# jorr3/Alphazero-4-player-chess

Measured on AMD Instinct MI355X. Metric: MCTS simulations/sec (whole node), 256 games×400 sims, 10-block ResNet, higher is better.
Workload: dtype fp16

## Files before the change

alphazero-4-player-chess_amd/csrc/fpc_fc.h:

```cpp
#pragma once
#include <hip/hip_runtime.h>

#include <type_traits>

#include "fpc_tower.h"

namespace fpc {

struct FcArgs {
  const uint16_t *X;
  const uint16_t *Wf;
  float *part;
  int Kp, Np, ksteps, Mtot;
  int G1, s1, s2;
  const int *n_live;
};

constexpr int FC_THREADS = 256;
constexpr int FC_XBUF = 256 * 64 * 2;
constexpr int FC_WRING = 16 * 1024;
constexpr int FC_LDS = 3 * FC_XBUF + 4 * FC_WRING;

__device__ __forceinline__ void fc_dma(const void *gsrc_uniform, uint32_t lane_off, uint32_t lds_addr_uniform) {
  uint32_t keep;
// ... 173 lines not shown
  f32x4_t acc[16][6];
  u32x4_t xr[4], wf[2][6];
  const std::integral_constant<int, 0> c0{};
  const std::integral_constant<int, 1> c1{};

  auto issue_x = [&](int s, int p) {
    const int sc = s < S ? s : S - 1;
    fc_dma(xbase + (long)p * xpiece + (long)sc * 128, xlane[p & 1],
           (uint32_t)__builtin_amdgcn_readfirstlane((s & 1) * FC_XBUF + (wave * 64 + p * 8) * 128));
  };
  auto issue_w2 = [&](int s, int j, int n0) {
    const int sc = s < S ? s : S - 1;
    fc_dma2_nt(wbase + (long)(2 * sc + j) * wk32 + n0 * 1024, wlane,
               (uint32_t)__builtin_amdgcn_readfirstlane(lds_w + ((s & 1) * 12 + j * 6 + n0) * 1024));
  };
  auto xfrag = [&](int slot, int t, const unsigned char *ab, int j) {
    xr[slot] = *reinterpret_cast<const u32x4_t *>(ab + lds_off<64>(t * 16 + (lane & 15), j * 4 + (lane >> 4)));
  };
  auto wfrag = [&](int b, int s, int j) {
#pragma unroll
    for (int n = 0; n < 6; ++n) wf[b][n] = *reinterpret_cast<const u32x4_t *>(wr + ((s & 1) * 12 + j * 6 + n) * 1024);
  };
  auto kstep = [&](auto j_c, auto z_c, int s) {
    constexpr int J = decltype(j_c)::value;
    constexpr bool Z = decltype(z_c)::value != 0;
    constexpr int CUR = J, NXT = J ^ 1;
    asm volatile("s_waitcnt vmcnt(20)" ::: "memory");
    const unsigned char *ab = smem + (s & 1) * FC_XBUF;
    const unsigned char *abn = J == 1 ? smem + ((s + 1) & 1) * FC_XBUF : ab;
    __builtin_amdgcn_sched_barrier(0);
    wfrag(NXT, J == 1 ? s + 1 : s, NXT);
    __builtin_amdgcn_sched_barrier(0);
#pragma unroll
    for (int t = 0; t < 16; ++t) {
#pragma unroll
      for (int n = 0; n < 6; ++n) {
        if (n < 4) fcw_mfma<DT, true, Z>(acc[t][n], wf[CUR][n], xr[t & 3]);
        else fcw_mfma<DT, false, Z>(acc[t][n], wf[CUR][n], xr[t & 3]);
      }
      __builtin_amdgcn_sched_barrier(0);
      if (J == 1 && t == 13) { asm volatile("s_waitcnt vmcnt(12)" ::: "memory"); __syncthreads(); }
      if (t + 3 < 16) xfrag((t + 3) & 3, t + 3, ab, J);
      else xfrag((t + 3) & 3, t + 3 - 16, abn, NXT);
      if (J == 0 && t < 8) issue_x(s + 1, t);
      if (J == 0 && (t == 8 || t == 10 || t == 12)) issue_w2(s + 2, 0, t - 8);
      if (J == 1 && (t == 2 || t == 6 || t == 10)) issue_w2(s + 2, 1, (t - 2) / 2);
      __builtin_amdgcn_sched_barrier(0);
    }
  };

#pragma unroll
  for (int p = 0; p < 8; ++p) issue_x(0, p);
#pragma unroll
  for (int st = 0; st < 2; ++st)
#pragma unroll
    for (int j = 0; j < 2; ++j) { issue_w2(st, j, 0); issue_w2(st, j, 2); issue_w2(st, j, 4); }
  asm volatile("s_waitcnt vmcnt(0)" ::: "memory");
  __syncthreads();
#pragma unroll
  for (int t = 0; t < 3; ++t) xfrag(t, t, smem, 0);
  wfrag(0, 0, 0);

  kstep(c0, c1, 0);
  kstep(c1, c0, 0);
#pragma unroll 1
  for (int s = 1; s < S; ++s) {
    kstep(c0, c0, s);
    kstep(c1, c0, s);
  }
  asm volatile("s_waitcnt vmcnt(0)" ::: "memory");
  asm volatile("s_nop 7\n\ts_nop 7\n\ts_nop 3" ::: "memory");

  float *out = g.part + ((long)id * g.Mtot + mrow0) * FCW_COLS;
#pragma unroll
  for (int t = 0; t < 16; ++t) {
    const int m = t * 16 + (lane & 15);
#pragma unroll
    for (int n = 0; n < 6; ++n)
      *reinterpret_cast<f32x4_t *>(out + (long)m * FCW_COLS + wave * 96 + n * 16 + (lane >> 4) * 4) = acc[t][n];
  }
}


template <bool LIVE = false>
__global__ void __launch_bounds__(256) k_fc_reduce(const float *part, const float *bias, int G1, int s1, int s2, int gw, int Mtot, int A,
                                                   int n_rows, const int *n_live, float *logits, float *stats) {
  __shared__ float red[8];
  const int q = blockIdx.x * 256 + threadIdx.x;
  const int m = blockIdx.y;
  if (m >= n_rows || (LIVE && m >= *n_live)) return;
  const bool valid = q * 4 < A;
  float4 v{0.f, 0.f, 0.f, 0.f};
  if (valid) {
    const int j = gw == 256 ? q >> 6 : (q * 4) / gw;
    const int col = q * 4 - j * gw;
    const int base = j < G1 ? j * s1 : G1 * s1 + (j - G1) * s2, cnt = j < G1 ? s1 : s2;
    v = *reinterpret_cast<const float4 *>(bias + q * 4);
    for (int k = 0; k < cnt; ++k) {
      const float4 p = *reinterpret_cast<const float4 *>(part + ((long)(base + k) * Mtot + m) * gw + col);
      v.x += p.x; v.y += p.y; v.z += p.z; v.w += p.w;
    }
    if (logits) *reinterpret_cast<float4 *>(logits + (long)m * A + q * 4) = v;
  }
  softmax_chunk_stats(v, valid, red, stats + ((long)m * SM_MAXCH + blockIdx.x) * SM_REC);
}

}
```

alphazero-4-player-chess_amd/csrc/fpc_nn.h:

```cpp
#pragma once
#include <hip/hip_runtime.h>

#include <algorithm>
#include <cstdlib>
#include <cstring>
#include <string>
#include <vector>

#include "fpc_tree_kernels.h"
#include "fpc_pack.h"
#include "fpc_tower.h"
#include "fpc_towerw.h"

namespace fpc {

typedef __attribute__((ext_vector_type(8))) __bf16 bf16x8_t;
typedef __attribute__((ext_vector_type(8))) _Float16 f16x8_t;
typedef __attribute__((ext_vector_type(16))) float f32x16_t;
typedef __attribute__((ext_vector_type(4))) uint32_t u32x4_t;
typedef __attribute__((ext_vector_type(2))) uint32_t u32x2_t;
typedef __attribute__((ext_vector_type(4))) float f32x4_t;

template <int DT>
struct E16;
// ... 276 lines not shown
            const u32x4_t x = xrow[q0 + 64 * u];
            a0 = Dot16<DT>::dot2(w[u][0], x[0], a0); a1 = Dot16<DT>::dot2(w[u][1], x[1], a1);
            a2 = Dot16<DT>::dot2(w[u][2], x[2], a2); a3 = Dot16<DT>::dot2(w[u][3], x[3], a3);
          }
        }
      }
      float a = (a0 + a1) + (a2 + a3);
      for (int off = 32; off >= 1; off >>= 1) a += __shfl_xor(a, off);
      if (lane == 0) ll[(size_t)g * FPC_MAX_MOVES + j] = bias[nsrc] + a;
    }
    p = pend;
  }
}

template <int DT>
__global__ void __launch_bounds__(64) k_value_tail(const uint16_t *Y, const float *w, float bias, int P, int R, int PP,
                                                   int n, float *out) {
  const int g = blockIdx.x;
  if (g >= n) return;
  const int lane = threadIdx.x & 63;
  float acc = 0.f;
  for (int idx = lane; idx < R * R * 32; idx += 64) {
    const int q = idx >> 5, ch = idx & 31;
    const long m = (long)g * PP + (q / R + 1) * P + (q % R + 1);
    acc += E16<DT>::to_f32(Y[m * 32 + ch]) * w[idx];
  }
  for (int off = 32; off >= 1; off >>= 1) acc += __shfl_xor(acc, off);
  if (lane == 0) out[g] = tanhf(acc + bias);
}

template <int DT>
__global__ void __launch_bounds__(64) k_nchw_to_grid(const float *x, int n, int R, int P, uint16_t *out) {
  const int g = blockIdx.x;
  if (g >= n) return;
  const int lane = threadIdx.x & 63, RR = R * R;
  for (int q = lane; q < RR; q += 64) {
    uint16_t *row = out + ((long)g * P * P + (q / R + 1) * P + (q % R + 1)) * 32;
    for (int c = 0; c < 32; ++c) row[c] = c < 24 ? E16<DT>::from_f32(x[((long)g * 24 + c) * RR + q]) : (uint16_t)0;
  }
}

struct BlobHeader {
  char magic[4];
  int32_t version, R, F, nblocks, dtype, A_ch, Np, Kp;
  int32_t fc_layout;
  int32_t pad[6];
};
static_assert(sizeof(BlobHeader) == 64, "header is 64 bytes");

struct ConvW {
  uint16_t *w = nullptr;
  float *b = nullptr;
  int cin = 0, cout_pad = 0;
};

struct NN {
  bool loaded = false;
  DevCfg dc{};
  int Gmax = 0, dtype = 0, F = 0, nblocks = 0, P = 0, PP = 0, Np = 0, Kp = 0, Mrows = 0, guard = 64, Gpad = 0;
  hipStream_t stream = nullptr;
  std::vector<void *> allocs;
  uint16_t *in16 = nullptr;
  uint16_t *act[3] = {nullptr, nullptr, nullptr};
  uint16_t *yv = nullptr;
  uint16_t *xfc = nullptr;
  float *d_logits = nullptr;
  float *d_stats = nullptr;
  float *d_value = nullptr;
  ConvW stem, pconv, vconv;
  std::vector<ConvW> c1, c2;
  uint16_t *fcw = nullptr;
  float *fcb = nullptr, *vw = nullptr;
  float *fc_part = nullptr;
  int fc_G1 = 0, fc_s1 = FC_SPLITK, fc_s2 = FC_SPLITK;
  int fc_layout = 1;
  int fc_gw = 256;
  unsigned char *towerW = nullptr;
  unsigned char *stemW = nullptr;
  float *towerB = nullptr;
  bool use_tower = false;
  int tower_waves = 8;
  bool tower_compact = true;
  bool tower_taploop = true;
  int towerw_rows = 1;
  bool use_towerw = false;
  void (*mark_fn)(void *, int) = nullptr;
  void *mark_ctx = nullptr;
  float vb = 0.f;
  bool attr_conv[2][3] = {{false, false, false}, {false, false, false}}, attr_tower[2] = {false, false}, attr_towerw[2] = {false, false}, attr_fc[2] = {false, false}, attr_gemv = false;

  template <class T>
  int dmalloc(T **p, size_t count, std::string *err) {
    void *q = nullptr;
    if (hipMalloc(&q, count * sizeof(T)) != hipSuccess) { *err = "hipMalloc failed in NN (" + std::to_string(count * sizeof(T)) + " bytes)"; return FPC_ENOMEM; }
    (void)hipMemset(q, 0, count * sizeof(T));
    allocs.push_back(q);
    *p = (T *)q;
    return 0;
  }

  int init(const DevCfg &c, int max_games, int nn_dtype, hipStream_t s, std::string *) {
    dc = c; Gmax = max_games; dtype = nn_dtype ? 1 : 0; stream = s;
    P = c.R + 2; PP = P * P;
    Mrows = ((max_games * PP + CONV_BM - 1) / CONV_BM) * CONV_BM;
    Gpad = ((max_games + 255) / 256) * 256;
    return 0;
  }
  void destroy() {
    for (void *p : allocs) (void)hipFree(p);
    allocs.clear();
    loaded = false;
    fcw2 = nullptr; d_ll = nullptr;
  }
  uint16_t *input16() { return in16 + (size_t)guard * 32; }
  const fpc_board *in_boards = nullptr;
  const int *in_leaf_slot = nullptr, *in_leaf_turn = nullptr;
  int in_board_stride = 0;
  bool takes_boards() const { return use_tower || use_towerw; }
  void set_board_input(const fpc_board *b, int stride, const int *slot, const int *turn) { in_boards = b; in_board_stride = stride; in_leaf_slot = slot; in_leaf_turn = turn; }
  const int *in_live_count = nullptr;
  void set_live_count(const int *n_live) { in_live_count = n_live; }
  uint16_t one16() const { return dtype ? 0x3C00 : 0x3F80; }
  float *logits() { return d_logits; }
  float *stats() { return d_stats; }
  float *value() { return d_value; }
  uint16_t *fcw2 = nullptr;
  float *d_ll = nullptr;
  float *legal_logits() { return d_ll; }

  static int plan_fcw(int Np, int Kp, int cus) { return pk_plan_fcw(Np, Kp, cus); }
  static_assert(PK_FCW_COLS == FCW_COLS && PK_FCW_MAXSPLIT == 2 * FC_SPLITK, "fpc_pack.h plans k_fcw's split with these");
  void plan_fc() {
    if (fc_layout == 2) { fc_G1 = Np / FCW_COLS; fc_s2 = fc_s1; return; }
    fc_s1 = FC_SPLITK;
    const int groups = Np / 256, ks = Kp / 16, mt = (Gmax + 255) / 256;
    fc_s2 = (ks % (2 * FC_SPLITK * 8) == 0 && ks / (2 * FC_SPLITK) / 4 >= 4) ? 2 * FC_SPLITK : FC_SPLITK;
    fc_G1 = groups;
    if (fc_s2 == FC_SPLITK) return;
    int cus = 256;
    hipDeviceProp_t prop;
    int dev = 0;
    (void)hipGetDevice(&dev);
    if (hipGetDeviceProperties(&prop, dev) == hipSuccess && prop.multiProcessorCount > 0) cus = prop.multiProcessorCount;
    long best = -1;
    std::vector<long> fin(cus);
    for (int g1 = groups; g1 >= 0; --g1) {
      std::fill(fin.begin(), fin.end(), 0L);
      for (int y = 0; y < mt; ++y)
        for (int id = 0, nb = g1 * FC_SPLITK + (groups - g1) * fc_s2; id < nb; ++id) {
          auto it = std::min_element(fin.begin(), fin.end());
          *it += id < g1 * FC_SPLITK ? 2 : 1;
        }
      const long span = *std::max_element(fin.begin(), fin.end());
      if (best < 0 || span < best) { best = span; fc_G1 = g1; }
    }
  }

  static int device_cus() {
    int cus = 256, dev = 0;
    hipDeviceProp_t prop;
    (void)hipGetDevice(&dev);
    if (hipGetDeviceProperties(&prop, dev) == hipSuccess && prop.multiProcessorCount > 0) cus = prop.multiProcessorCount;
    return cus;
  }
  int check_geom(int gF, int gnblocks, int gNp, int gKp, int glayout, int *split, std::string *err) const {
    return pk_check_geom(gF, gnblocks, gNp, gKp, glayout, dc.A, device_cus(), split, err);
  }
  bool same_geom(int gF, int gnblocks, int gNp, int gKp, int glayout) const {
    return loaded && F == gF && nblocks == gnblocks && Np == gNp && Kp == gKp && fc_layout == glayout;
  }
  int alloc_net(int gF, int gnblocks, int gNp, int gKp, int glayout, int split, std::string *err) {
    destroy();
    F = gF; nblocks = gnblocks; Np = gNp; Kp = gKp;
    fc_layout = glayout;
    fc_gw = fc_layout == 2 ? FCW_COLS : 256;
    if (fc_layout == 2) fc_s1 = split;
    int rc = 0;
    auto conv = [&](ConvW &cw, int cin, int cout_pad) -> int {
      cw.cin = cin; cw.cout_pad = cout_pad;
      if ((rc = dmalloc(&cw.w, (size_t)9 * cout_pad * cin, err))) return rc;
      return dmalloc(&cw.b, (size_t)cout_pad, err);
    };
    const int Fp = (F + GEMM_BN - 1) / GEMM_BN * GEMM_BN;
    if ((rc = conv(stem, 32, Fp))) return rc;
    c1.assign(nblocks, ConvW()); c2.assign(nblocks, ConvW());
    for (int i = 0; i < nblocks; ++i) { if ((rc = conv(c1[i], F, Fp)) || (rc = conv(c2[i], F, Fp))) return rc; }
    if ((rc = conv(pconv, F, 128))) return rc;
    if ((rc = conv(vconv, F, 128))) return rc;
    if ((rc = dmalloc(&fcw, (size_t)Np * Kp, err)) || (rc = dmalloc(&fcb, (size_t)Np, err))) return rc;
    if ((rc = dmalloc(&vw, (size_t)dc.RR * 32, err))) return rc;
    const size_t rows = (size_t)Mrows + 2 * guard;
    if ((rc = dmalloc(&in16, rows * 32, err))) return rc;
    for (auto &a : act) if ((rc = dmalloc(&a, rows * F, err))) return rc;
    if ((rc = dmalloc(&yv, rows * 32, err))) return rc;
    if ((rc = dmalloc(&xfc, (size_t)Gpad * Kp, err))) return rc;
    if ((rc = dmalloc(&fc_part, (size_t)2 * FC_SPLITK * Gpad * Np, err))) return rc;
    plan_fc();
    if ((rc = dmalloc(&d_logits, (size_t)Gmax * dc.A, err))) return rc;
    if ((rc = dmalloc(&d_stats, (size_t)Gmax * SM_MAXCH * SM_REC, err))) return rc;
    if ((rc = dmalloc(&d_value, (size_t)Gmax, err))) return rc;
    use_tower = use_towerw = false;
    const bool dev = getenv("FPC_DEV_KNOBS") && atoi(getenv("FPC_DEV_KNOBS")) != 0;
    auto knob = [dev](const char *name, int dflt) { const char *v = dev ? getenv(name) : nullptr; return v ? atoi(v) : dflt; };
    const bool no_tower = knob("FPC_NO_TOWER", 0) != 0;
    tower_waves = knob("FPC_TOWER_WAVES", 8);
    tower_compact = knob("FPC_TOWER_COMPACT", 1) != 0;
    tower_taploop = knob("FPC_TOWER_TAPLOOP", 1) != 0;
    if (F == 256 && !no_tower) {
      use_towerw = true;
      towerw_rows = knob("FPC_TOWERW_ROWS", 1);
    } else if (F == 128 && !no_tower) {
      const int kw = knob("FPC_TOWERW", -1);
      use_towerw = kw < 0 ? dc.R != 14 : kw != 0;
      use_tower = !use_towerw;
    }
    const int layers = 2 * nblocks + 2;
    if (use_towerw) {
      const int slab = tww_slab(F), ksn = F / 32;
      if ((rc = dmalloc(&towerW, ((size_t)layers * 9 * ksn + TWW_PAD_SLABS) * slab, err)) || (rc = dmalloc(&stemW, (size_t)9 * slab, err)) ||
          (rc = dmalloc(&towerB, (size_t)layers * 256, err))) return rc;
    } else if (use_tower) {
      if ((rc = dmalloc(&towerW, (size_t)(layers * 9 + 3) * TW_TAP, err)) || (rc = dmalloc(&stemW, (size_t)9 * TW_STEM_TAP, err)) ||
          (rc = dmalloc(&towerB, (size_t)layers * 256, err))) return rc;
    }
    return 0;
  }
  std::vector<ConvW *> convs_in_blob_order() {
    std::vector<ConvW *> v{&stem};
    for (int i = 0; i < nblocks; ++i) { v.push_back(&c1[i]); v.push_back(&c2[i]); }
    v.push_back(&pconv); v.push_back(&vconv);
    return v;
  }
  int finish_weights(std::string *err) {
    if (use_towerw) {
      const int slab = tww_slab(F), ksn = F / 32, tiles = F / 16;
      auto prep = [&](const ConvW &cw, int layer) {
        hipLaunchKernelGGL(k_towerw_prep, dim3((9 * ksn * tiles * 64 + 255) / 256), dim3(256), 0, stream, (const uint16_t *)cw.w,
                           towerW + (size_t)layer * 9 * ksn * slab, 9, cw.cout_pad, F, tiles);
        (void)hipMemcpyAsync(towerB + (size_t)layer * 256, cw.b, (size_t)std::min(cw.cout_pad, F) * 4, hipMemcpyDeviceToDevice, stream);
      };
      for (int i = 0; i < nblocks; ++i) { prep(c1[i], 2 * i); prep(c2[i], 2 * i + 1); }
      prep(vconv, 2 * nblocks);
      prep(pconv, 2 * nblocks + 1);
      hipLaunchKernelGGL(k_towerw_prep, dim3((9 * tiles * 64 + 255) / 256), dim3(256), 0, stream, (const uint16_t *)stem.w, stemW, 9, stem.cout_pad, 32, tiles);
    } else if (use_tower) {
      auto prep = [&](const ConvW &cw, int layer) {
        hipLaunchKernelGGL(k_tower_prep, dim3((9 * 128 * 16 + 255) / 256), dim3(256), 0, stream, (const uint16_t *)cw.w,
                           towerW + (size_t)layer * 9 * TW_TAP, 9, 128);
        (void)hipMemcpyAsync(towerB + (size_t)layer * 256, cw.b, 128 * 4, hipMemcpyDeviceToDevice, stream);
      };
      for (int i = 0; i < nblocks; ++i) { prep(c1[i], 2 * i); prep(c2[i], 2 * i + 1); }
      prep(vconv, 2 * nblocks);
      prep(pconv, 2 * nblocks + 1);
      hipLaunchKernelGGL(k_tower_prep, dim3((9 * 128 * 4 + 255) / 256), dim3(256), 0, stream, (const uint16_t *)stem.w, stemW, 9, 32);
    }
    if (fcw2) launch_unfrag();
    if (hipStreamSynchronize(stream) != hipSuccess || hipGetLastError() != hipSuccess) { *err = use_towerw ? "k_towerw_prep failed" : use_tower ? "k_tower_prep failed" : "weight load failed"; return FPC_ENODEVICE; }
    loaded = true;
    return 0;
  }

  int load(const void *blob, uint64_t nbytes, std::string *err) {
    if (nbytes < sizeof(BlobHeader)) { *err = "weight blob too small"; return FPC_EWEIGHTS; }
    BlobHeader h;
    memcpy(&h, blob, sizeof(h));
    if (memcmp(h.magic, "FPCW", 4) || h.version != 3) { *err = "bad weight blob magic/version (this engine reads version 3; version 2 carried the retired 32x32x16 policy-Linear order: export again)"; return FPC_EWEIGHTS; }
    if (h.R != dc.R || h.A_ch != dc.A_ch) { *err = "weight blob is for a different board size"; return FPC_EWEIGHTS; }
    if (h.dtype != dtype) { *err = "weight blob dtype differs from engine nn_dtype"; return FPC_EWEIGHTS; }
    int fcw_split = 0, rc = 0;
    if ((rc = check_geom(h.F, h.nblocks, h.Np, h.Kp, h.fc_layout, &fcw_split, err))) return rc;
    if ((rc = alloc_net(h.F, h.nblocks, h.Np, h.Kp, h.fc_layout, fcw_split, err))) return rc;
    const unsigned char *base = (const unsigned char *)blob;
    uint64_t off = sizeof(BlobHeader);
    auto take = [&](void *dev, uint64_t bytes) -> int {
      off = (off + 63) & ~63ull;
      if (off + bytes > nbytes) { *err = "weight blob truncated"; return FPC_EWEIGHTS; }
      if (hipMemcpy(dev, base + off, bytes, hipMemcpyHostToDevice) != hipSuccess) { *err = "weight upload failed"; return FPC_ENODEVICE; }
      off += bytes;
      return 0;
    };
    for (ConvW *cw : convs_in_blob_order())
      if ((rc = take(cw->w, (uint64_t)9 * cw->cout_pad * cw->cin * 2)) || (rc = take(cw->b, (uint64_t)cw->cout_pad * 4))) return rc;
    if ((rc = take(fcw, (uint64_t)Np * Kp * 2)) || (rc = take(fcb, (uint64_t)Np * 4))) return rc;
    if ((rc = take(vw, (uint64_t)dc.RR * 32 * 4))) return rc;
    off = (off + 63) & ~63ull;
    if (off + 4 > nbytes) { *err = "weight blob truncated"; return FPC_EWEIGHTS; }
    memcpy(&vb, base + off, 4);
    return finish_weights(err);
  }

// ... 79 lines not shown
#undef FPC_TWW_ATTR1
          aw = true;
        }
        const int mtw = tww_mt(dc.R);
        if (mtw < 2 || mtw > 7) { *err = "k_towerw: board size outside 8..14"; return FPC_EINVAL; }
#define FPC_TWW_GO(F_, MT_) hipLaunchKernelGGL((k_towerw<DT, F_, MT_>), dim3(n), dim3(TWW_THREADS), tww_lds(F_), stream, t)
#define FPC_TWW_GOS(F_) switch (mtw) { case 2: FPC_TWW_GO(F_, 2); break; case 3: FPC_TWW_GO(F_, 3); break; case 4: FPC_TWW_GO(F_, 4); break; \
                                       case 5: FPC_TWW_GO(F_, 5); break; case 6: FPC_TWW_GO(F_, 6); break; default: FPC_TWW_GO(F_, 7); break; }
        const int tiles = tww_tiles(dc.R);
        const bool onerow = tiles <= 4 || (F == 256 && towerw_rows != 2);
#define FPC_TWW_GO1(F_, MT_) hipLaunchKernelGGL((k_towerw<DT, F_, MT_, true>), dim3(n), dim3(TWW_THREADS), tww_lds(F_), stream, t)
        if (onerow && F == 128) FPC_TWW_GO1(128, 4);
        else if (onerow) {
          switch (tiles) {
            case 4: FPC_TWW_GO1(256, 4); break;   case 6: FPC_TWW_GO1(256, 6); break;   case 7: FPC_TWW_GO1(256, 7); break;
            case 8: FPC_TWW_GO1(256, 8); break;   case 9: FPC_TWW_GO1(256, 9); break;   case 11: FPC_TWW_GO1(256, 11); break;
            default: FPC_TWW_GO1(256, 13); break;
          }
        } else if (F == 256) { FPC_TWW_GOS(256) } else { FPC_TWW_GOS(128) }
#undef FPC_TWW_GO1
#undef FPC_TWW_GOS
#undef FPC_TWW_GO
      } else if (mt == 3 && tower_waves == 8) hipLaunchKernelGGL((k_tower<DT, 3, false, 8>), dim3(n), dim3(512), TW_LDS, stream, t);
      else if (mt == 3) hipLaunchKernelGGL((k_tower<DT, 3, false, 4>), dim3(n), dim3(256), TW_LDS, stream, t);
      else if (mt == 5 && tower_waves == 8) hipLaunchKernelGGL((k_tower<DT, 5, false, 8>), dim3(n), dim3(512), TW_LDS, stream, t);
      else if (mt == 5) hipLaunchKernelGGL((k_tower<DT, 5, false, 4>), dim3(n), dim3(256), TW_LDS, stream, t);
      else if (P != 16 && tower_waves == 8) hipLaunchKernelGGL((k_tower<DT, 7, false, 8>), dim3(n), dim3(512), TW_LDS, stream, t);
      else if (P != 16) hipLaunchKernelGGL((k_tower<DT, 7, false, 4>), dim3(n), dim3(256), TW_LDS, stream, t);
      else if (tower_waves == 8 && tower_compact && dc.R == 14 && tower_taploop) hipLaunchKernelGGL((k_towerc<DT, true>), dim3(n), dim3(512), TW_LDS, stream, t);
      else if (tower_waves == 8 && tower_compact && dc.R == 14) hipLaunchKernelGGL((k_towerc<DT, false>), dim3(n), dim3(512), TW_LDS, stream, t);
      else if (tower_waves == 8) hipLaunchKernelGGL((k_tower<DT, 7, true, 8>), dim3(n), dim3(512), TW_LDS, stream, t);
      else hipLaunchKernelGGL((k_tower<DT, 7, true, 4>), dim3(n), dim3(256), TW_LDS, stream, t);
      const hipError_t le = hipGetLastError();
      if (le != hipSuccess) { *err = std::string("k_tower launch failed: ") + hipGetErrorString(le); return FPC_ENODEVICE; }
#if defined(TW_STAMPS) || defined(TWW_STAMPS)
      if (getenv("FPC_TW_STAMPS_FILE")) {
        unsigned long long h[2 * 8 * 16];
        (void)hipStreamSynchronize(stream);
        (void)hipMemcpy(h, t.stamps, sizeof(h), hipMemcpyDeviceToHost);
        if (FILE *f = fopen(getenv("FPC_TW_STAMPS_FILE"), "w")) {
          for (int i = 0; i < 2 * 8 * 16; ++i) fprintf(f, "%llu%c", h[i], i % 16 == 15 ? '\n' : ' ');
          fclose(f);
        }
      }
#endif
    } else if ((rc = conv(stem, in16, 32, nullptr, act[0], F, F, 0))) return rc;
    const bool fused = use_tower || use_towerw;
    for (int i = 0; i < nblocks && !fused; ++i) {
      const int t1 = (cur + 1) % 3, t2 = (cur + 2) % 3;
      if ((rc = conv(c1[i], act[cur], F, nullptr, act[t1], F, F, 0))) return rc;
      if ((rc = conv(c2[i], act[t1], F, act[cur], act[t2], F, F, 0))) return rc;
      cur = t2;
    }
    if (!fused) {
      if ((rc = conv(pconv, act[cur], F, nullptr, xfc, Kp, dc.A_ch, 1))) return rc;
      if ((rc = conv(vconv, act[cur], F, nullptr, yv, 32, 24, 0))) return rc;
    }
    if (mark_fn) mark_fn(mark_ctx, 2);
#if defined(TW_STRIP) && (TW_STRIP & 128)
    if (false) {
#else
    if (logits_out) {
#endif
      FcArgs f{};
      f.X = xfc; f.Wf = fcw; f.part = fc_part; f.Kp = Kp; f.Np = Np; f.ksteps = Kp / 16; f.Mtot = Gpad;
      f.G1 = fc_G1; f.s1 = fc_s1; f.s2 = fc_s2;
      f.n_live = in_live_count;
      const int mtiles = (n + 255) / 256;
      const int blocks = fc_G1 * fc_s1 + (Np / fc_gw - fc_G1) * fc_s2;
      bool &fattr = attr_fc[DT];
      if (!fattr) {
        (void)hipFuncSetAttribute(reinterpret_cast<const void *>(&k_fc16<DT>), hipFuncAttributeMaxDynamicSharedMemorySize, FC_LDS);
        (void)hipFuncSetAttribute(reinterpret_cast<const void *>(&k_fcw<DT>), hipFuncAttributeMaxDynamicSharedMemorySize, FCW_LDS);
        (void)hipFuncSetAttribute(reinterpret_cast<const void *>(&k_fc16<DT, true>), hipFuncAttributeMaxDynamicSharedMemorySize, FC_LDS);
        (void)hipFuncSetAttribute(reinterpret_cast<const void *>(&k_fcw<DT, true>), hipFuncAttributeMaxDynamicSharedMemorySize, FCW_LDS);
        fattr = true;
      }
      const bool live = in_live_count != nullptr;
      if (fc_layout == 2 && live) hipLaunchKernelGGL((k_fcw<DT, true>), dim3(blocks, mtiles), dim3(FC_THREADS), FCW_LDS, stream, f);
      else if (fc_layout == 2) hipLaunchKernelGGL((k_fcw<DT>), dim3(blocks, mtiles), dim3(FC_THREADS), FCW_LDS, stream, f);
      else if (live) hipLaunchKernelGGL((k_fc16<DT, true>), dim3(blocks, mtiles), dim3(FC_THREADS), FC_LDS, stream, f);
      else hipLaunchKernelGGL((k_fc16<DT>), dim3(blocks, mtiles), dim3(FC_THREADS), FC_LDS, stream, f);
      float *const dense_out = skip_dense ? (float *)nullptr : logits_out;
      if (live)
        hipLaunchKernelGGL(k_fc_reduce<true>, dim3((dc.A / 4 + 255) / 256, n), dim3(256), 0, stream, (const float *)fc_part, (const float *)fcb,
                           fc_G1, fc_s1, fc_s2, fc_gw, Gpad, dc.A, n, in_live_count, dense_out, d_stats);
      else
        hipLaunchKernelGGL(k_fc_reduce<false>, dim3((dc.A / 4 + 255) / 256, n), dim3(256), 0, stream, (const float *)fc_part, (const float *)fcb,
                           fc_G1, fc_s1, fc_s2, fc_gw, Gpad, dc.A, n, in_live_count, dense_out, d_stats);
      const hipError_t le = hipGetLastError();
      if (le != hipSuccess) { *err = std::string("k_fc launch failed: ") + hipGetErrorString(le); return FPC_ENODEVICE; }
    }
    if (!fused) hipLaunchKernelGGL((k_value_tail<DT>), dim3(n), dim3(64), 0, stream, (const uint16_t *)(yv + (size_t)guard * 32),
                       (const float *)vw, vb, P, dc.R, PP, n, value_out);
    if (hipGetLastError() != hipSuccess) { *err = "k_value_tail launch failed"; return FPC_ENODEVICE; }
    return 0;
  }

  bool skip_dense = false;
  int forward(int n, bool dense_logits, std::string *err) {
    skip_dense = !dense_logits;
    const int rc = dtype ? forward_t<1>(n, d_logits, d_value, err) : forward_t<0>(n, d_logits, d_value, err);
    skip_dense = false;
    return rc;
  }
  static_assert(2 * FC_SPLITK <= LOGIT_MAX_SLABS, "logit_at() requests at most LOGIT_MAX_SLABS slabs per column");
  LogitSrc logit_src(bool dense) const {
    if (dense) return LogitSrc{d_logits, nullptr, nullptr, 0, 0, 0, 0, 256};
    return LogitSrc{nullptr, fc_part, fcb, fc_G1, fc_s1, fc_s2, Gpad, fc_gw};
  }
  void launch_unfrag() {
    const long chunks = (long)Np * (Kp / 8);
    if (dtype) hipLaunchKernelGGL((k_fc_unfrag<1>), dim3((unsigned)((chunks + 255) / 256)), dim3(256), 0, stream, (const uint16_t *)fcw, fcw2, Np, Kp);
    else hipLaunchKernelGGL((k_fc_unfrag<0>), dim3((unsigned)((chunks + 255) / 256)), dim3(256), 0, stream, (const uint16_t *)fcw, fcw2, Np, Kp);
  }
  int ensure_legal_head(std::string *err) {
    if (fcw2) return 0;
    if (Gmax > GEMV_MAXG) { *err = "legal-only policy head supports at most " + std::to_string(GEMV_MAXG) + " games per engine"; return FPC_EINVAL; }
    int rc;
    if ((rc = dmalloc(&fcw2, (size_t)Np * Kp, err)) || (rc = dmalloc(&d_ll, (size_t)Gmax * FPC_MAX_MOVES, err))) return rc;
    launch_unfrag();
    if (hipGetLastError() != hipSuccess) { *err = "k_fc_unfrag launch failed"; return FPC_ENODEVICE; }
    return 0;
  }
  int forward_legal(int n, const Tree &t, std::string *err) {
    int rc = ensure_legal_head(err);
    if (rc) return rc;
    if ((rc = dtype ? forward_t<1>(n, nullptr, d_value, err) : forward_t<0>(n, nullptr, d_value, err))) return rc;
    const size_t lds = (size_t)Kp * 2;
    bool &attr = attr_gemv;
    if (!attr) {
      (void)hipFuncSetAttribute(reinterpret_cast<const void *>(&k_policy_gemv<0>), hipFuncAttributeMaxDynamicSharedMemorySize, 64 * 1024);
      (void)hipFuncSetAttribute(reinterpret_cast<const void *>(&k_policy_gemv<1>), hipFuncAttributeMaxDynamicSharedMemorySize, 64 * 1024);
      attr = true;
    }
    if (lds > 64 * 1024) { *err = "legal-only policy head: activation row does not fit LDS"; return FPC_EINVAL; }
    const int blocks = 768;
    if (dtype) hipLaunchKernelGGL((k_policy_gemv<1>), dim3(blocks), dim3(GEMV_THREADS), lds, stream, dc, t, n, (const uint16_t *)xfc, (const uint16_t *)fcw2, (const float *)fcb, Kp, d_ll);
    else hipLaunchKernelGGL((k_policy_gemv<0>), dim3(blocks), dim3(GEMV_THREADS), lds, stream, dc, t, n, (const uint16_t *)xfc, (const uint16_t *)fcw2, (const float *)fcb, Kp, d_ll);
    if (hipGetLastError() != hipSuccess) { *err = "k_policy_gemv launch failed"; return FPC_ENODEVICE; }
    return 0;
  }
  int forward_external(const float *enc, int n, float *logits_out, float *value_out, std::string *err) {
    if (dtype) hipLaunchKernelGGL((k_nchw_to_grid<1>), dim3(n), dim3(64), 0, stream, enc, n, dc.R, P, input16());
    else hipLaunchKernelGGL((k_nchw_to_grid<0>), dim3(n), dim3(64), 0, stream, enc, n, dc.R, P, input16());
    int rc = dtype ? forward_t<1>(n, logits_out, value_out, err) : forward_t<0>(n, logits_out, value_out, err);
    if (rc) return rc;
    if (hipStreamSynchronize(stream) != hipSuccess) { *err = "NN forward failed"; return FPC_ENODEVICE; }
    return 0;
  }
};

}
```

alphazero-4-player-chess_amd/csrc/fpc_tower.h:

```cpp
#pragma once
#include <hip/hip_runtime.h>

#include <type_traits>

#include "fpc_tree_kernels.h"

namespace fpc {

typedef __attribute__((ext_vector_type(8))) __bf16 t_bf16x8;
typedef __attribute__((ext_vector_type(8))) _Float16 t_f16x8;
typedef __attribute__((ext_vector_type(4))) float t_f32x4;
typedef __attribute__((ext_vector_type(2))) float t_f32x2;
typedef __attribute__((ext_vector_type(4))) uint32_t t_u32x4;
typedef __attribute__((ext_vector_type(2))) uint32_t t_u32x2;
typedef __attribute__((ext_vector_type(2))) short t_i16x2;

template <int DT>
struct M16;
template <>
struct M16<0> {
  static __device__ __forceinline__ t_f32x4 mfma(t_u32x4 a, t_u32x4 b, t_f32x4 c) {
    return __builtin_amdgcn_mfma_f32_16x16x32_bf16(__builtin_bit_cast(t_bf16x8, a), __builtin_bit_cast(t_bf16x8, b), c, 0, 0, 0);
  }
  static __device__ __forceinline__ uint32_t pack2(float lo, float hi) {
// ... 74 lines not shown
}
__device__ __forceinline__ void tw_dma_4k(const unsigned char *gsrc_uniform, uint32_t lane_off, uint32_t lds_addr_uniform) {
  uint32_t keep;
  asm volatile(
      "s_mov_b32 %0, m0\n\ts_mov_b32 m0, %3\n\ts_nop 0\n\t"
      "global_load_lds_dwordx4 %1, %2\n\ts_add_u32 m0, m0, 0x400\n\tv_add_u32 %1, 0x400, %1\n\t"
      "global_load_lds_dwordx4 %1, %2\n\ts_add_u32 m0, m0, 0x400\n\tv_add_u32 %1, 0x400, %1\n\t"
      "global_load_lds_dwordx4 %1, %2\n\ts_add_u32 m0, m0, 0x400\n\tv_add_u32 %1, 0x400, %1\n\t"
      "global_load_lds_dwordx4 %1, %2\n\t"
      "s_mov_b32 m0, %0"
      : "=&s"(keep), "+v"(lane_off) : "s"(gsrc_uniform), "s"(lds_addr_uniform) : "memory", "scc");
}
template <int OFF>
__device__ __forceinline__ void tw_dma_piece(const unsigned char *gsrc_uniform, uint32_t lane_off) {
  asm volatile("global_load_lds_dwordx4 %0, %1 offset:%2" : : "v"(lane_off), "s"(gsrc_uniform), "i"(OFF) : "memory");
}
__device__ __forceinline__ void tw_set_m0(uint32_t lds_addr_uniform) {
  asm volatile("s_mov_b32 m0, %0\n\ts_nop 0" : : "s"(lds_addr_uniform) : "memory");
}
__device__ __forceinline__ void tw_dma_256(const unsigned char *gsrc_uniform, uint32_t lane_off, uint32_t lds_addr_uniform) {
  uint32_t keep;
  asm volatile("s_mov_b32 %0, m0\n\ts_mov_b32 m0, %3\n\ts_nop 0\n\tglobal_load_lds_dword %1, %2\n\ts_mov_b32 m0, %0"
               : "=&s"(keep) : "v"(lane_off), "s"(gsrc_uniform), "s"(lds_addr_uniform) : "memory");
}

#ifdef TW_STAMPS
#define TW_STAMP(GT, I)                                                                                       \
  do {                                                                                                        \
    if (g.stamps && blockIdx.x == 0 && ((GT) == TW_STAMPS || (GT) == TW_STAMPS + 1)) {                        \
      const unsigned long long t_ = __builtin_amdgcn_s_memtime();                                             \
      if (lane == 0) g.stamps[(((GT) - TW_STAMPS) * 8 + wave) * 16 + (I)] = t_;                               \
    }                                                                                                         \
  } while (0)
#else
#define TW_STAMP(GT, I) do {} while (0)
#endif
#ifndef TW_AHEAD
#define TW_AHEAD 2
#endif
#ifndef TW_LOADERS
#define TW_LOADERS 1
#endif
#ifndef TW_STAGGER
#define TW_STAGGER 3
#endif
#ifndef TW_STRIP
#define TW_STRIP 0
#endif
#ifndef TWC_LOADER_TILES
#define TWC_LOADER_TILES 6
#endif

#ifndef TWC_STAGGER
#define TWC_STAGGER 2
#endif

template <int DT, int MT, bool FAST, int NW, int LOAD, bool CMP = false, bool TU = false>
__device__ __forceinline__ void tw_body(const TowerArgs &g) {
  static_assert(!CMP || (!FAST && NW == 8 && TW_LOADERS == 1 && MT == (LOAD == 2 ? TWC_LOADER_TILES : 13 - TWC_LOADER_TILES)), "compact form: 8 waves, 13 row tiles");
  static_assert(!TU || (CMP && TW_STAGGER != 0 && TWC_STAGGER >= 1 && TWC_STAGGER <= 3), "tap-specialised loop: compact form with the burst stream");
  constexpr int CR = 14, CZ = 16;
  constexpr int TB0 = LOAD == 2 ? 0 : TWC_LOADER_TILES;
  constexpr int NT = NW * 64;
  constexpr int WN = NW / 2;
  constexpr int CT = 8 / WN;
  constexpr int PIECES = 4 * LOAD;
  constexpr int DMA_PER_WAVE = PIECES * 1024;
  constexpr int MID = PIECES == 8 ? 4096 : 0;
  constexpr bool STREAM = TW_AHEAD == 2 && !(TW_STAGGER != 0 && NW == 8 && TW_LOADERS == 1);
  constexpr int STAG = (NW == 8 && TW_LOADERS == 1 && LOAD == 0) ? (TU ? TWC_STAGGER : TW_STAGGER) : 0;
  extern __shared__ __attribute__((aligned(16))) unsigned char smem[];
  unsigned char *const img = smem + TW_IMG0;
  unsigned char *const ring = smem + TW_RING;
  const float *const biasbuf = reinterpret_cast<const float *>(smem + TW_BIAS);
  float *const vred = reinterpret_cast<float *>(smem + TW_VRED);
  fpc_board *const lboard = reinterpret_cast<fpc_board *>(smem + TW_BOARD);
  const int tid = threadIdx.x, lane = tid & 63;
  const int wave = __builtin_amdgcn_readfirstlane(tid >> 6);
  const int wm = wave / WN, wn = wave % WN;
  const int li = lane & 15, lq = lane >> 4;
  const int game = blockIdx.x;
  const int P = g.P, NR = g.NR;

  int slot = 0, rot_k = 0;
  if (g.boards) {
    slot = g.leaf_slot[game];
    if (slot < 0) return;
    rot_k = first_leaf_turn(g.leaf_slot, g.leaf_turn, g.n_games);
  }

  const int rbase = CMP ? CZ + TB0 * 16 + li : (g.T0 + wm * MT) * 16 + li;
  uint32_t inmask = 0;
#pragma unroll
  for (int mt = 0; mt < MT; ++mt) {
    const int r = rbase + 16 * mt;
    if (CMP) {
      if (r - CZ < CR * CR) inmask |= 1u << mt;
    } else {
      const int pi = r / P, pj = r - pi * P;
      if (r < g.PP && pi >= 1 && pi <= g.R && pj >= 1 && pj <= g.R) inmask |= 1u << mt;
    }
  }
  auto colmask = [](int mt, int dx) -> uint64_t {
    uint32_t m16 = 0;
    for (int i = 0; i < 16; ++i)
      if (dx != 0 && ((TB0 + mt) * 16 + i) % CR == (dx < 0 ? 0 : CR - 1)) m16 |= 1u << i;
    const uint32_t m32 = m16 * 0x10001u;
    return ((uint64_t)m32 << 32) | m32;
  };
  auto lane_select = [](uint32_t a, uint32_t b, uint64_t m) -> uint32_t {
    uint32_t r;
    asm("v_cndmask_b32_e64 %0, %1, %2, %3" : "=v"(r) : "v"(a), "v"(b), "s"(m));
    return r;
  };
  const int bq = (lq >> 1) * 256 + (lq & 1) * 128;
  const int apart = (li >> 3) * 2048 + (li & 7) * 16 + bq;
  const int apart_s = (li >> 3) * 512 + (li & 7) * 16 + bq;
  const int cb64 = wn * (CT * 16);
  const int cb16 = (wn & 1) * 16;
  const bool vactive = wn < 2;

  for (int c = tid; c < (TW_IMG0 + TW_IMG) / 16; c += NT) reinterpret_cast<t_u32x4 *>(smem)[c] = t_u32x4{0u, 0u, 0u, 0u};
  unsigned char *const enc = smem + TW_ENC;
  const int enc_bytes = CMP ? 240 * 64 : ((NR + 7) >> 3) * 512;
  for (int c = tid; c < enc_bytes / 16; c += NT) reinterpret_cast<t_u32x4 *>(enc)[c] = t_u32x4{0u, 0u, 0u, 0u};
  {
    const t_u32x4 *src = reinterpret_cast<const t_u32x4 *>(g.Wstem);
    t_u32x4 *dst = reinterpret_cast<t_u32x4 *>(ring);
    for (int c = tid; c < 9 * TW_STEM_TAP / 16; c += NT) dst[c] = src[c];
  }
  t_f32x4 bst[CT];
#pragma unroll
  for (int ct = 0; ct < CT; ++ct) bst[ct] = *reinterpret_cast<const t_f32x4 *>(g.bstem + cb64 + ct * 16 + 4 * lq);
  __syncthreads();
  if (g.boards) {
    constexpr int WPB = (int)(sizeof(fpc_board) / 4);
    if (tid < WPB) reinterpret_cast<uint32_t *>(lboard)[tid] =
        reinterpret_cast<const uint32_t *>(g.boards + (size_t)game * g.board_stride + slot)[tid];
    __syncthreads();
    if (g.rules & FPC_RULES_ROTATION) rot_k = lboard->turn;
    for (int r = tid; r < (CMP ? CR * CR : g.PP); r += NT) {
      const int pi = CMP ? r / CR + 1 : r / P, pj = CMP ? r % CR + 1 : r - pi * P;
      if (pi < 1 || pi > g.R || pj < 1 || pj > g.R) continue;
      const uint8_t p = lboard->sq[rot90_src(g.R, rot_k, pi - 1, pj - 1)];
      if (!present(p)) continue;
      const int plane = piece_plane(p, lboard->turn, g.rules);
      *reinterpret_cast<uint16_t *>(enc + tw_lay(4, CMP ? CZ + r : r, plane >> 3) + (plane & 7) * 2) = g.one16;
    }
  } else if (CMP) {
    const uint16_t *src = g.in16 + (size_t)game * g.PP * 32;
    for (int c = tid; c < CR * CR * 4; c += NT) {
      const int q = c >> 2, j = c & 3;
      *reinterpret_cast<t_u32x4 *>(enc + tw_lay(4, CZ + q, j)) =
          *reinterpret_cast<const t_u32x4 *>(src + ((size_t)(q / CR + 1) * P + q % CR + 1) * 32 + j * 8);
    }
  } else {
    const uint16_t *src = g.in16 + (size_t)game * g.PP * 32;
    for (int c = tid; c < NR * 4; c += NT) {
      const int r = c >> 2, j = c & 3;
      *reinterpret_cast<t_u32x4 *>(enc + tw_lay(4, r, j)) = *reinterpret_cast<const t_u32x4 *>(src + (size_t)r * 32 + j * 8);
    }
  }
  __syncthreads();

  t_f32x4 acc[MT][CT];
  t_u32x2 res[MT][CT];

  auto brow = [&](int mt, int shift) -> int {
    int r = rbase + 16 * mt + shift;
    r = r < 0 ? r + NR : r;
    r = r >= NR ? r - NR : r;
    return r;
  };

#pragma unroll
  for (int tap = 0; tap < 9; ++tap) {
    const int shift = (tap / 3 - 1) * (CMP ? CR : P) + (tap % 3 - 1);
    t_u32x4 fa[CT], fb[MT];
#pragma unroll
    for (int ct = 0; ct < CT; ++ct)
      fa[ct] = *reinterpret_cast<const t_u32x4 *>(ring + tap * TW_STEM_TAP + (cb64 + ct * 16) * 64 + apart_s);
#pragma unroll
    for (int mt = 0; mt < MT; ++mt) {
      const int r = CMP ? (int)lane_select((uint32_t)(rbase + 16 * mt + shift), (uint32_t)((rbase + shift) & 7), colmask(mt, tap % 3 - 1)) : brow(mt, shift);
      fb[mt] = *reinterpret_cast<const t_u32x4 *>(enc + (r >> 3) * 512 + (r & 7) * 16 + bq);
    }
#pragma unroll
    for (int mt = 0; mt < MT; ++mt)
#pragma unroll
      for (int ct = 0; ct < CT; ++ct) acc[mt][ct] = M16<DT>::mfma(fa[ct], fb[mt], tap == 0 ? bst[ct] : acc[mt][ct]);
  }
  __syncthreads();

  const int total = (g.L + 2) * 9;
  const uint32_t dma_lane = (uint32_t)lane * 16u;
  const int lw = LOAD == 2 ? (wave & 3) : wave;
  auto issue_bias = [&](int T) {
    if (T % 9 == 0 && T < total && wave < 4) {
      const int l = T / 9;
      tw_dma_256(reinterpret_cast<const unsigned char *>(g.bt + (size_t)l * 256 + wave * 64), (uint32_t)lane * 4u,
                 (uint32_t)__builtin_amdgcn_readfirstlane(TW_BIAS + ((l & 1) * 256 + wave * 64) * 4));
    }
  };
  auto issue_tap = [&](int T) {
    issue_bias(T);
    if (LOAD == 0 || (TW_STRIP & 4)) return;
    const unsigned char *src = g.Wt + (size_t)T * TW_TAP + lw * DMA_PER_WAVE;
    const uint32_t dst = (uint32_t)__builtin_amdgcn_readfirstlane(TW_RING + (T % 3) * TW_TAP + lw * DMA_PER_WAVE);
    if (PIECES == 8) tw_dma_8k(src, dma_lane, dst);
    else tw_dma_4k(src, dma_lane, dst);
  };
  const unsigned char *dsrc = g.Wt;
  auto open_tap = [&](int T) {
    issue_bias(T);
    if (LOAD == 0) return;
    dsrc = g.Wt + (size_t)T * TW_TAP + lw * DMA_PER_WAVE + MID;
    tw_set_m0((uint32_t)__builtin_amdgcn_readfirstlane(TW_RING + (T % 3) * TW_TAP + lw * DMA_PER_WAVE + MID));
  };
  auto piece = [&](auto i_c) {
    constexpr int I = decltype(i_c)::value;
    if (LOAD != 0) tw_dma_piece<I * 1024 - MID>(dsrc, dma_lane);
  };
// ... 331 lines not shown
```

Measured before the change: 499,600.

## Overlap tower prologue global loads and unroll FC split-K reduce loads

The tower kernel prologue now issues the stem-weight, bias, leaf-slot and board loads into registers up front, before the LDS zeroing. It finds the first live leaf's turn with a wave ballot instead of a serial scan, stores everything to LDS afterwards and drops one __syncthreads. The FC reduce kernel now issues all split-K partial loads at once in an unrolled, predicated form so they are in flight together; the old serial loop is kept behind a dev knob. This adds register pressure from the held weights and the partial-sum array, and an early return now happens after the shared zeroing, with no barrier after it.

```diff
diff --git a/alphazero-4-player-chess_amd/csrc/fpc_fc.h b/alphazero-4-player-chess_amd/csrc/fpc_fc.h
--- a/alphazero-4-player-chess_amd/csrc/fpc_fc.h
+++ b/alphazero-4-player-chess_amd/csrc/fpc_fc.h
@@ -279,7 +279,7 @@
 }
 
 
-template <bool LIVE = false>
+template <bool LIVE = false, bool SERIAL = false>
 __global__ void __launch_bounds__(256) k_fc_reduce(const float *part, const float *bias, int G1, int s1, int s2, int gw, int Mtot, int A,
                                                    int n_rows, const int *n_live, float *logits, float *stats) {
   __shared__ float red[8];
@@ -292,10 +292,27 @@
     const int j = gw == 256 ? q >> 6 : (q * 4) / gw;
     const int col = q * 4 - j * gw;
     const int base = j < G1 ? j * s1 : G1 * s1 + (j - G1) * s2, cnt = j < G1 ? s1 : s2;
-    v = *reinterpret_cast<const float4 *>(bias + q * 4);
-    for (int k = 0; k < cnt; ++k) {
-      const float4 p = *reinterpret_cast<const float4 *>(part + ((long)(base + k) * Mtot + m) * gw + col);
-      v.x += p.x; v.y += p.y; v.z += p.z; v.w += p.w;
+    const float *const p0 = part + ((long)base * Mtot + m) * gw + col;
+    const long pitch = (long)Mtot * gw;
+    if (SERIAL) {
+      v = *reinterpret_cast<const float4 *>(bias + q * 4);
+      for (int k = 0; k < cnt; ++k) {
+        const float4 p = *reinterpret_cast<const float4 *>(p0 + k * pitch);
+        v.x += p.x; v.y += p.y; v.z += p.z; v.w += p.w;
+      }
+    } else {
+      float4 p[2 * FC_SPLITK];
+      v = *reinterpret_cast<const float4 *>(bias + q * 4);
+#pragma unroll
+      for (int k = 0; k < 2 * FC_SPLITK; ++k) {
+        p[k] = float4{0.f, 0.f, 0.f, 0.f};
+        if (k < cnt) p[k] = *reinterpret_cast<const float4 *>(p0 + k * pitch);
+      }
+#pragma unroll
+      for (int k = 0; k < 2 * FC_SPLITK; ++k) {
+        v.x = k < cnt ? v.x + p[k].x : v.x; v.y = k < cnt ? v.y + p[k].y : v.y;
+        v.z = k < cnt ? v.z + p[k].z : v.z; v.w = k < cnt ? v.w + p[k].w : v.w;
+      }
     }
     if (logits) *reinterpret_cast<float4 *>(logits + (long)m * A + q * 4) = v;
   }
diff --git a/alphazero-4-player-chess_amd/csrc/fpc_nn.h b/alphazero-4-player-chess_amd/csrc/fpc_nn.h
--- a/alphazero-4-player-chess_amd/csrc/fpc_nn.h
+++ b/alphazero-4-player-chess_amd/csrc/fpc_nn.h
@@ -382,6 +382,7 @@
   int tower_waves = 8;
   bool tower_compact = true;
   bool tower_taploop = true;
+  bool fc_reduce_serial = false;
   int towerw_rows = 1;
   bool use_towerw = false;
   void (*mark_fn)(void *, int) = nullptr;
@@ -506,6 +507,7 @@
     tower_waves = knob("FPC_TOWER_WAVES", 8);
     tower_compact = knob("FPC_TOWER_COMPACT", 1) != 0;
     tower_taploop = knob("FPC_TOWER_TAPLOOP", 1) != 0;
+    fc_reduce_serial = knob("FPC_FC_REDUCE_SERIAL", 0) != 0;
     if (F == 256 && !no_tower) {
       use_towerw = true;
       towerw_rows = knob("FPC_TOWERW_ROWS", 1);
@@ -751,12 +753,10 @@
       else if (live) hipLaunchKernelGGL((k_fc16<DT, true>), dim3(blocks, mtiles), dim3(FC_THREADS), FC_LDS, stream, f);
       else hipLaunchKernelGGL((k_fc16<DT>), dim3(blocks, mtiles), dim3(FC_THREADS), FC_LDS, stream, f);
       float *const dense_out = skip_dense ? (float *)nullptr : logits_out;
-      if (live)
-        hipLaunchKernelGGL(k_fc_reduce<true>, dim3((dc.A / 4 + 255) / 256, n), dim3(256), 0, stream, (const float *)fc_part, (const float *)fcb,
-                           fc_G1, fc_s1, fc_s2, fc_gw, Gpad, dc.A, n, in_live_count, dense_out, d_stats);
-      else
-        hipLaunchKernelGGL(k_fc_reduce<false>, dim3((dc.A / 4 + 255) / 256, n), dim3(256), 0, stream, (const float *)fc_part, (const float *)fcb,
-                           fc_G1, fc_s1, fc_s2, fc_gw, Gpad, dc.A, n, in_live_count, dense_out, d_stats);
+      auto *const reduce = live ? (fc_reduce_serial ? &k_fc_reduce<true, true> : &k_fc_reduce<true, false>)
+                                : (fc_reduce_serial ? &k_fc_reduce<false, true> : &k_fc_reduce<false, false>);
+      hipLaunchKernelGGL(reduce, dim3((dc.A / 4 + 255) / 256, n), dim3(256), 0, stream, (const float *)fc_part, (const float *)fcb,
+                         fc_G1, fc_s1, fc_s2, fc_gw, Gpad, dc.A, n, in_live_count, dense_out, d_stats);
       const hipError_t le = hipGetLastError();
       if (le != hipSuccess) { *err = std::string("k_fc launch failed: ") + hipGetErrorString(le); return FPC_ENODEVICE; }
     }
diff --git a/alphazero-4-player-chess_amd/csrc/fpc_tower.h b/alphazero-4-player-chess_amd/csrc/fpc_tower.h
--- a/alphazero-4-player-chess_amd/csrc/fpc_tower.h
+++ b/alphazero-4-player-chess_amd/csrc/fpc_tower.h
@@ -180,12 +180,16 @@
   const int game = blockIdx.x;
   const int P = g.P, NR = g.NR;
 
-  int slot = 0, rot_k = 0;
+  constexpr int SW = 9 * TW_STEM_TAP / 16 / NT;
+  static_assert(SW * NT * 16 == 9 * TW_STEM_TAP, "the stem's weights divide among the threads");
+  int slot = 0, rot_k = 0, scan_slot = -1, scan_turn = 0;
   if (g.boards) {
     slot = g.leaf_slot[game];
-    if (slot < 0) return;
-    rot_k = first_leaf_turn(g.leaf_slot, g.leaf_turn, g.n_games);
-  }
+    if (lane < g.n_games) { scan_slot = g.leaf_slot[lane]; scan_turn = g.leaf_turn[lane]; }
+  }
+  t_u32x4 sw[SW];
+#pragma unroll
+  for (int i = 0; i < SW; ++i) sw[i] = reinterpret_cast<const t_u32x4 *>(g.Wstem)[tid + i * NT];
 
   const int rbase = CMP ? CZ + TB0 * 16 + li : (g.T0 + wm * MT) * 16 + li;
   uint32_t inmask = 0;
@@ -218,24 +222,31 @@
   const int cb16 = (wn & 1) * 16;
   const bool vactive = wn < 2;
 
-  for (int c = tid; c < (TW_IMG0 + TW_IMG) / 16; c += NT) reinterpret_cast<t_u32x4 *>(smem)[c] = t_u32x4{0u, 0u, 0u, 0u};
+  t_f32x4 bst[CT];
+#pragma unroll
+  for (int ct = 0; ct < CT; ++ct) bst[ct] = *reinterpret_cast<const t_f32x4 *>(g.bstem + cb64 + ct * 16 + 4 * lq);
+
+  static_assert(TW_BOARD % 16 == 0 && sizeof(fpc_board) % 16 == 0, "the board covers whole 16-byte pieces");
+  for (int c = tid; c < (TW_IMG0 + TW_IMG) / 16; c += NT)
+    if (!(g.boards && c >= TW_BOARD / 16 && c < (TW_BOARD + (int)sizeof(fpc_board)) / 16)) reinterpret_cast<t_u32x4 *>(smem)[c] = t_u32x4{0u, 0u, 0u, 0u};
   unsigned char *const enc = smem + TW_ENC;
   const int enc_bytes = CMP ? 240 * 64 : ((NR + 7) >> 3) * 512;
   for (int c = tid; c < enc_bytes / 16; c += NT) reinterpret_cast<t_u32x4 *>(enc)[c] = t_u32x4{0u, 0u, 0u, 0u};
-  {
-    const t_u32x4 *src = reinterpret_cast<const t_u32x4 *>(g.Wstem);
-    t_u32x4 *dst = reinterpret_cast<t_u32x4 *>(ring);
-    for (int c = tid; c < 9 * TW_STEM_TAP / 16; c += NT) dst[c] = src[c];
-  }
-  t_f32x4 bst[CT];
-#pragma unroll
-  for (int ct = 0; ct < CT; ++ct) bst[ct] = *reinterpret_cast<const t_f32x4 *>(g.bstem + cb64 + ct * 16 + 4 * lq);
+  if (slot < 0) return;
+  constexpr int WPB = (int)(sizeof(fpc_board) / 4);
+  uint32_t bword = 0;
+  if (g.boards) {
+    if (tid < WPB) bword = reinterpret_cast<const uint32_t *>(g.boards + (size_t)game * g.board_stride + slot)[tid];
+    asm volatile("" : "+v"(scan_slot), "+v"(scan_turn) : : "memory");
+    const unsigned long long bal = __ballot(scan_slot >= 0);
+    rot_k = bal ? wave_read(scan_turn, (int)__ffsll((long long)bal) - 1)
+                : (g.n_games > 64 ? first_leaf_turn(g.leaf_slot, g.leaf_turn, g.n_games) : 0);
+  }
+#pragma unroll
+  for (int i = 0; i < SW; ++i) reinterpret_cast<t_u32x4 *>(ring)[tid + i * NT] = sw[i];
+  if (g.boards && tid < WPB) reinterpret_cast<uint32_t *>(lboard)[tid] = bword;
   __syncthreads();
   if (g.boards) {
-    constexpr int WPB = (int)(sizeof(fpc_board) / 4);
-    if (tid < WPB) reinterpret_cast<uint32_t *>(lboard)[tid] =
-        reinterpret_cast<const uint32_t *>(g.boards + (size_t)game * g.board_stride + slot)[tid];
-    __syncthreads();
     if (g.rules & FPC_RULES_ROTATION) rot_k = lboard->turn;
     for (int r = tid; r < (CMP ? CR * CR : g.PP); r += NT) {
       const int pi = CMP ? r / CR + 1 : r / P, pj = CMP ? r % CR + 1 : r - pi * P;
```

Result: no change. 501,700, median of 6 (+0.4%).
